# SunBangjie/FYP-BidirectionalPathTracer

Measured on AMD Instinct MI355X. Metric: Mrays/s + RMSE vs the scalar oracle, BDPT pass, Sponza-class scene 1920x1080 depth 8, higher is better.
Workload: dtype f32

## Files before the change

### fyp-bidirectionalpathtracer_amd/csrc/device_scene.hpp

```cpp
#pragma once
#include "device_math.hpp"
#include "kernels.h"

namespace bdpt {
#define BD __device__ __forceinline__

struct f4 {
  float x, y, z, w;
};
BD f4 lerp4(f4 a, f4 b, float s) {
  return f4{a.x + (b.x - a.x) * s, a.y + (b.y - a.y) * s, a.z + (b.z - a.z) * s, a.w + (b.w - a.w) * s};
}
typedef __attribute__((address_space(1))) const uint32_t gU32;
typedef __attribute__((address_space(1), aligned(4))) const unsigned long long gU64a4;
BD void texelRow(const uint8_t* px, uint32_t w, int iy, int ix0, int ix1, uint32_t& a, uint32_t& b) {
  gU32* row = (gU32*)px + (size_t)iy * w;
  const unsigned long long q = *(gU64a4*)(row + ix0);
  a = (uint32_t)q;
  b = (uint32_t)(q >> 32);
  if (ix1 != ix0 + 1) b = row[ix1];
}
BD f4 texel(const SceneDev& S, const TexDev& t, uint32_t p) {
  f4 r;
  if (t.srgb) {
    r.x = S.sc->srgbLut[p & 0xffu];
    r.y = S.sc->srgbLut[(p >> 8) & 0xffu];
    r.z = S.sc->srgbLut[(p >> 16) & 0xffu];
  } else {
    r.x = (float)(p & 0xffu) / 255.0f;
    r.y = (float)((p >> 8) & 0xffu) / 255.0f;
    r.z = (float)((p >> 16) & 0xffu) / 255.0f;
  }
  r.w = (float)(p >> 24) / 255.0f;
  return r;
}
BD f4 sampleBilinearT(const SceneDev& S, const TexDev& t, float u, float v) {
  float x = u * (float)t.w - 0.5f;
  float y = v * (float)t.h - 0.5f;
  float x0 = floorf(x), y0 = floorf(y);
  float fx = x - x0, fy = y - y0;
  int ix0 = wrapT((int)x0, (int)t.w, (t.pow2 & kTexPow2W) != 0u), iy0 = wrapT((int)y0, (int)t.h, (t.pow2 & kTexPow2H) != 0u);
  int ix1 = wrapNext(ix0, (int)t.w), iy1 = wrapNext(iy0, (int)t.h);
  uint32_t p00, p10, p01, p11;
  texelRow(t.px, t.w, iy0, ix0, ix1, p00, p10);
  texelRow(t.px, t.w, iy1, ix0, ix1, p01, p11);
  f4 t00 = texel(S, t, p00), t10 = texel(S, t, p10);
  f4 t01 = texel(S, t, p01), t11 = texel(S, t, p11);
  return lerp4(lerp4(t00, t10, fx), lerp4(t01, t11, fx), fy);
}
BD f4 sampleBilinear(const SceneDev& S, int texId, float u, float v) { return sampleBilinearT(S, S.textures[texId], u, v); }
BD f4 sampleTexture(const SceneDev& S, int texId, float u, float v, f4 factor, uint32_t mode) {
  if (mode == BDPT_CHANNEL_UNUSED) return f4{0, 0, 0, 0};
  if (mode == BDPT_CHANNEL_CONST || texId < 0) return factor;
  return sampleBilinear(S, texId, u, v);
}
BD f4 sampleTextureT(const SceneDev& S, const TexDev& t, int texId, float u, float v, f4 factor, uint32_t mode) {
  if (mode == BDPT_CHANNEL_UNUSED) return f4{0, 0, 0, 0};
  if (mode == BDPT_CHANNEL_CONST || texId < 0) return factor;
  return sampleBilinearT(S, t, u, v);
}

struct MatDev {
  f4 baseColor, specular;
  f3 emissive;
  float alphaThreshold, IoR;
  uint32_t flags;
  int texBase, texSpec, texEmis, texNorm;
};
BD MatDev loadMaterial(const SceneDev& S, uint32_t id) {
  const float4* m = reinterpret_cast<const float4*>(S.materials + id);
  float4 a = m[0], b = m[1], c = m[2], d = m[3];
  MatDev r;
  r.baseColor = f4{a.x, a.y, a.z, a.w};
  r.specular = f4{b.x, b.y, b.z, b.w};
  r.emissive = mk(c.x, c.y, c.z);
  r.alphaThreshold = c.w;
  r.IoR = d.x;
  r.flags = __float_as_uint(d.y);
  uint32_t t0 = __float_as_uint(d.z), t1 = __float_as_uint(d.w);
  r.texBase = (int)(int16_t)(t0 & 0xffffu);
  r.texSpec = (int)(int16_t)(t0 >> 16);
  r.texEmis = (int)(int16_t)(t1 & 0xffffu);
  r.texNorm = (int)(int16_t)(t1 >> 16);
  return r;
}

BD uint32_t alphaQuad(const float4& a2, const float4& a3, float u, float v, float& fx, float& fy) {
  const int tw = (int)__float_as_uint(a2.y), th = (int)__float_as_uint(a2.z);
  const uint32_t pow2 = __float_as_uint(a2.w);
  gU32* px = (gU32*)(((unsigned long long)__float_as_uint(a3.y) << 32) | (unsigned long long)__float_as_uint(a3.x));
  const float x = u * (float)tw - 0.5f, y = v * (float)th - 0.5f;
  const float x0 = floorf(x), y0 = floorf(y);
  fx = x - x0;
  fy = y - y0;
  const int ix0 = wrapT((int)x0, tw, (pow2 & kTexPow2W) != 0u), iy0 = wrapT((int)y0, th, (pow2 & kTexPow2H) != 0u);
  return px[(size_t)iy0 * tw + (size_t)ix0];
}
BD bool alphaTestFails(const SceneDev& S, uint32_t rec, float bu, float bv) {
  const float4* r = S.alphaRecs + (size_t)rec * 4;
  const float4 a0 = r[0], a1 = r[1], a2 = r[2], a3 = r[3];
  const uint32_t mode = __float_as_uint(a2.x);
  float alpha = 0.0f;
  if (mode == 1u) {
    alpha = a1.w;
  } else if (mode == 2u) {
    float u = 0, v = 0;
    const float b0 = 1.0f - bu - bv;
    u += a0.x * b0;
    v += a0.y * b0;
    u += a0.z * bu;
    v += a0.w * bu;
    u += a1.x * bv;
    v += a1.y * bv;
    float fx, fy;
    const uint32_t q = alphaQuad(a2, a3, u, v, fx, fy);
    const float t00 = (float)(q & 0xffu) / 255.0f, t10 = (float)((q >> 8) & 0xffu) / 255.0f;
    const float t01 = (float)((q >> 16) & 0xffu) / 255.0f, t11 = (float)(q >> 24) / 255.0f;
    const float top = t00 + (t10 - t00) * fx, bot = t01 + (t11 - t01) * fx;
    alpha = top + (bot - top) * fy;
  }
  return alpha < a1.z;
}

struct AlphaIn {
  float4 a0, a1, a2, a3;
};
BD void alphaTexels(const AlphaIn& r, float bu, float bv, bool run, float& fx, float& fy, float& t00, float& t10, float& t01, float& t11) {
  fx = fy = t00 = t10 = t01 = t11 = 0.0f;
  if (!run || __float_as_uint(r.a2.x) != 2u) return;
  float u = 0, v = 0;
  const float b0 = 1.0f - bu - bv;
  u += r.a0.x * b0;
  v += r.a0.y * b0;
  u += r.a0.z * bu;
  v += r.a0.w * bu;
  u += r.a1.x * bv;
  v += r.a1.y * bv;
  const uint32_t q = alphaQuad(r.a2, r.a3, u, v, fx, fy);
  t00 = (float)(q & 0xffu);
  t10 = (float)((q >> 8) & 0xffu);
  t01 = (float)((q >> 16) & 0xffu);
  t11 = (float)(q >> 24);
}
BD bool alphaVerdict(const AlphaIn& r, float fx, float fy, float t00, float t10, float t01, float t11) {
  const uint32_t mode = __float_as_uint(r.a2.x);
  float alpha = 0.0f;
  if (mode == 1u) {
    alpha = r.a1.w;
  } else if (mode == 2u) {
    const float w00 = t00 / 255.0f, w10 = t10 / 255.0f, w01 = t01 / 255.0f, w11 = t11 / 255.0f;
    const float top = w00 + (w10 - w00) * fx, bot = w01 + (w11 - w01) * fx;
    alpha = top + (bot - top) * fy;
  }
  return alpha < r.a1.z;
}
BD void alphaTestFails2(const SceneDev& S, bool need0, uint32_t rec0, float u0, float v0, bool need1, uint32_t rec1, float u1, float v1,
                        bool& fail0, bool& fail1) {
  AlphaIn r0, r1;
  r0.a0 = r0.a1 = r0.a2 = r0.a3 = r1.a0 = r1.a1 = r1.a2 = r1.a3 = make_float4(0.0f, 0.0f, 0.0f, 0.0f);
  if (need0) {
    const float4* p = S.alphaRecs + (size_t)rec0 * 4;
    r0.a0 = p[0];
    r0.a1 = p[1];
    r0.a2 = p[2];
    r0.a3 = p[3];
  }
  if (need1) {
    const float4* p = S.alphaRecs + (size_t)rec1 * 4;
    r1.a0 = p[0];
    r1.a1 = p[1];
    r1.a2 = p[2];
    r1.a3 = p[3];
  }
  float fx0, fy0, a00, a10, a01, a11, fx1, fy1, b00, b10, b01, b11;
  alphaTexels(r0, u0, v0, need0, fx0, fy0, a00, a10, a01, a11);
  alphaTexels(r1, u1, v1, need1, fx1, fy1, b00, b10, b01, b11);
  fail0 = need0 && alphaVerdict(r0, fx0, fy0, a00, a10, a01, a11);
  fail1 = need1 && alphaVerdict(r1, fx1, fy1, b00, b10, b01, b11);
}

struct Shading {
  f3 posW, V, N, diffuse, specular, emissive;
  float opacity, linearRoughness, roughness, IoR;
};
template <bool NMAP>
BD Shading shadeHit(const SceneDev& S, uint32_t prim, float bu, float bv, f3 camPosW) {
  const float4* r = S.shade + (size_t)prim * kShadeRecF4;
  const float4 r0 = r[0], r1 = r[1], r2 = r[2], r3 = r[3], r4 = r[4], r5 = r[5], r6 = r[6];
  const float b0 = 1.0f - bu - bv;
  float u = 0, v = 0;
  f3 normalW = mk(0), posW = mk(0);
  u += r1.z * b0;
  v += r1.w * b0;
  normalW = normalW + mk(r0.w, r1.x, r1.y) * b0;
  posW = posW + mk(r0.x, r0.y, r0.z) * b0;
  u += r3.z * bu;
  v += r3.w * bu;
  normalW = normalW + mk(r2.w, r3.x, r3.y) * bu;
  posW = posW + mk(r2.x, r2.y, r2.z) * bu;
  u += r5.z * bv;
  v += r5.w * bv;
  normalW = normalW + mk(r4.w, r5.x, r5.y) * bv;
  posW = posW + mk(r4.x, r4.y, r4.z) * bv;
  normalW = normalize(normalW);

  const uint32_t matId = __float_as_uint(r6.x);
  const MatDev m = loadMaterial(S, matId);
  const TexDev tBase = S.matTex[(size_t)matId * 4], tSpec = S.matTex[(size_t)matId * 4 + 1], tEmis = S.matTex[(size_t)matId * 4 + 2];
  Shading sd;
  f4 base = sampleTextureT(S, tBase, m.texBase, u, v, m.baseColor, BDPT_FLAG_DIFFUSE_TYPE(m.flags));
  sd.opacity = m.baseColor.w;
  sd.posW = posW;
  sd.V = normalize(camPosW - posW);
  sd.N = normalize(normalW);
  f4 spec = sampleTextureT(S, tSpec, m.texSpec, u, v, m.specular, BDPT_FLAG_SPECULAR_TYPE(m.flags));
  f3 baseRgb = mk(base.x, base.y, base.z);
  if (BDPT_FLAG_SHADING_MODEL(m.flags) == BDPT_SHADING_MODEL_METAL_ROUGH) {
    sd.diffuse = lerp3(baseRgb, mk(0), spec.z);
    sd.specular = lerp3(mk(0.04f), baseRgb, spec.z);
    sd.linearRoughness = spec.y;
  } else {
    sd.diffuse = baseRgb;
    sd.specular = mk(spec.x, spec.y, spec.z);
    sd.linearRoughness = 1.0f - spec.w;
  }
  sd.linearRoughness = maxf(0.08f, sd.linearRoughness);
  sd.roughness = sd.linearRoughness * sd.linearRoughness;
  f4 em = sampleTextureT(S, tEmis, m.texEmis, u, v, f4{m.emissive.x, m.emissive.y, m.emissive.z, 1.0f}, BDPT_FLAG_EMISSIVE_TYPE(m.flags));
  sd.emissive = mk(em.x, em.y, em.z);
  sd.IoR = m.IoR;
  const bool doubleSided = BDPT_FLAG_DOUBLE_SIDED(m.flags) != 0;
  if (NMAP) {
    const uint32_t mapType = BDPT_FLAG_NORMAL_MAP_TYPE(m.flags);
    if (mapType != BDPT_NORMAL_MAP_UNUSED && m.texNorm >= 0 && S.hasBitangents) {
      f3 bitW = mk(0);
      const float bw[3] = {b0, bu, bv};
#pragma unroll
      for (int i = 0; i < 3; i++) {
        uint32_t vi = S.indices[(size_t)prim * 3 + i];
        bitW = bitW + ld3(S.bitangents + (size_t)vi * 3) * bw[i];
      }
      bitW = normalize(bitW);
      f3 B = normalize(bitW - sd.N * dot(bitW, sd.N));
      f3 T = normalize(cross(B, sd.N));
      f4 mp = sampleBilinear(S, m.texNorm, u, v);
      f3 mapN;
      if (mapType == BDPT_NORMAL_MAP_RGB) {
        mapN = normalize(mk(mp.x, mp.y, mp.z) * 2.0f - mk(1.0f));
      } else {
        float nx = mp.x * 2.0f - 1.0f, ny = mp.y * 2.0f - 1.0f;
        float nz = saturate(mp.x * mp.x + mp.y * mp.y);
        nz = sqrtf(1.0f - nz);
        mapN = normalize(mk(nx, ny, nz));
      }
      sd.N = T * mapN.x + B * mapN.y + sd.N * mapN.z;
    }
  }
  float NdotV = dot(sd.N, sd.V);
  if (NdotV <= 0.0f && doubleSided) sd.N = -sd.N;
  return sd;
}

BD void primaryRay(const bdpt_camera& cam, const bdpt_gbuffer_params& gp, uint32_t x, uint32_t y, uint32_t W, uint32_t H, f3& o, f3& d) {
  const f3 U = ld3(cam.cameraU), V = ld3(cam.cameraV), Wv = ld3(cam.cameraW), camPos = ld3(cam.posW);
  float pcx = ((float)x + gp.pixelJitter[0]) / (float)W;
  float pcy = ((float)y + gp.pixelJitter[1]) / (float)H;
  float ndx = 2.0f * pcx + -1.0f;
  float ndy = -2.0f * pcy + 1.0f;
  f3 rayDir = U * ndx + V * ndy + Wv;
  rayDir = rayDir / length(Wv);
  f3 focalPoint = camPos + rayDir * gp.focalLen;
  uint32_t randSeed = initRand(x + y * W, gp.frameCount);
  float r0 = nextRand(randSeed);
  float r1 = nextRand(randSeed);
  float sn, cs;
  det_sincos2pi(r0, sn, cs);
  float lr = gp.lensRadius * r1;
  float lu = cs * lr, lv = sn * lr;
  f3 randomOrig = camPos + normalize(U) * lu + normalize(V) * lv;
  o = gp.useThinLens ? randomOrig : camPos;
  d = normalize(gp.useThinLens ? (focalPoint - randomOrig) : rayDir);
}

#undef BD
}
```

### fyp-bidirectionalpathtracer_amd/csrc/device_trace.hpp

```cpp
#pragma once
#include "bvh.h"
#include "device_scene.hpp"

namespace bdpt {
#define BD __device__ __forceinline__
#define BDPT_ONE_WAVE_PER_GROUP()               \
  do {                                          \
    if (blockDim.x != (unsigned)kWave) return;  \
  } while (0)

struct Hit {
  int prim;
  float t, u, v;
  uint32_t rec;
};

constexpr int kDone = (int)0x80000000;

struct TravState {
  f3 o, d, idir;
  uint32_t neg;
  float tmin, tmax;
  int cur, sp;
  Hit best;
// ... 266 lines not shown
}

template <int MODE, bool COUNT>
BD Hit traverse(const SceneDev& S, f3 o, f3 d, float tmin, float tmax, int* stk, uint32_t& nNodes, uint32_t& nTris) {
  uint32_t nAlpha = 0;
  TravState T;
  travInit(T, o, d, tmin, tmax);
  while (T.cur != kDone) {
    while (T.cur >= 0) {
      if (COUNT) nNodes++;
      nodeStep<(MODE != 2) ? 1 : 0>(S, T, stk);
    }
    if (T.cur == kDone) break;
    if (leafStep<MODE, COUNT>(S, T, nTris, nAlpha)) break;
    T.cur = travPop<kStackEntries>(S, T, stk);
  }
  return T.best;
}

constexpr uint32_t kNoHint = 0xFFFFFFFFu;
BD bool recOccludes(const SceneDev& S, uint32_t rec, f3 o, f3 d, float tmin, float tmax) {
  if (rec >= S.numRecs) return false;
  TravState T;
  travInit(T, o, d, tmin, tmax);
  if (T.cur == kDone) return false;
  const float4* tp = reinterpret_cast<const float4*>(S.recs) + (size_t)rec * kRecF4;
  const TriCand k = triGeom<2>(T, tp[0], tp[1], tp[2]);
  if (!k.ok) return false;
  if ((k.flags & 1u) && alphaTestFails(S, k.aux, k.u, k.v)) return false;
  return true;
}
BD uint32_t cubeTexel(f3 v, uint32_t res) {
  const float ax = fabsf(v.x), ay = fabsf(v.y), az = fabsf(v.z);
  uint32_t face;
  float ma, uc, vc;
  if (ax >= ay && ax >= az) {
    face = v.x < 0.0f ? 1u : 0u;
    ma = ax;
    uc = v.y;
    vc = v.z;
  } else if (ay >= az) {
    face = v.y < 0.0f ? 3u : 2u;
    ma = ay;
    uc = v.x;
    vc = v.z;
  } else {
    face = v.z < 0.0f ? 5u : 4u;
    ma = az;
    uc = v.x;
    vc = v.y;
  }
  if (!(ma > 0.0f)) return kNoHint;
  const float fr = (float)res;
  const float fu = (uc / ma * 0.5f + 0.5f) * fr, fv = (vc / ma * 0.5f + 0.5f) * fr;
  const uint32_t iu = fu >= fr ? res - 1u : (uint32_t)(fu < 0.0f ? 0.0f : fu), iv = fv >= fr ? res - 1u : (uint32_t)(fv < 0.0f ? 0.0f : fv);
  return (face * res + iv) * res + iu;
}
BD uint32_t lightHint(const SceneDev& S, int light, f3 lightPos, f3 pos) {
  if (!S.lightMap) return kNoHint;
  const uint32_t t = cubeTexel(pos - lightPos, S.lightMapRes);
  if (t == kNoHint) return kNoHint;
  return S.lightMap[(size_t)light * 6u * S.lightMapRes * S.lightMapRes + t];
}

BD void addCount(DevCounters* c, int idx, uint32_t n) {
  if (n) atomicAdd(&c->v[blockIdx.x % kCounterShards][idx], (unsigned long long)n);
}
BD void waveAddCount(DevCounters* c, int idx, uint32_t n) {
  uint32_t v = n;
#pragma unroll
  for (int off = 32; off > 0; off >>= 1) v += (uint32_t)__shfl_xor((int)v, off);
  if ((threadIdx.x & 63u) == 0u && v) atomicAdd(&c->v[blockIdx.x % kCounterShards][idx], (unsigned long long)v);
}

#ifndef BDPT_LEAF_WAIT
#define BDPT_LEAF_WAIT 1
#endif
#ifndef BDPT_LEAF_WAIT_FRAC8
#define BDPT_LEAF_WAIT_FRAC8 4
#endif
#ifndef BDPT_NODE_BURST
#define BDPT_NODE_BURST 3
#endif
#ifndef BDPT_REFILL_IDLE
#define BDPT_REFILL_IDLE 16
#endif
constexpr int kRefillIdle = BDPT_REFILL_IDLE;

struct RayQueue {
  const float* rays;
  uint32_t cap;
  uint32_t subCap;
  uint32_t numSub;
  const uint32_t* count;
  uint32_t* head;
};

template <bool COUNT>
__global__ __launch_bounds__(kWave) void trace_shadow_kernel(SceneDev S, RayQueue Q, uint8_t* __restrict__ vis, DevCounters* counters,
                                                             float shadowTmin) {
  BDPT_ONE_WAVE_PER_GROUP();
  __shared__ int s_stack[kStackLds * kWave];
  int* stk = s_stack + threadIdx.x;
  const int lane = (int)(threadIdx.x & 63u);
  bool has = false, exhausted = false;
  uint32_t rid = 0;
  TravState T;
  T.cur = kDone;
  uint32_t nNodes = 0, nTris = 0, nAlpha = 0;
  int maxSp = 0;
  uint32_t q = blockIdx.x % Q.numSub, tried = 0, chunkPos = 0, chunkEnd = 0, chunk = kFetchChunk;
  const uint32_t wavesPerList = (gridDim.x + Q.numSub - 1) / Q.numSub;
  for (;;) {
    const unsigned long long idleMask = __ballot(!has);
    const int idle = __popcll(idleMask);
    if (!exhausted && idle >= kRefillIdle) {
      while (chunkPos >= chunkEnd && !exhausted) {
        const uint32_t nq = Q.count[q * kCursorStride];
        uint32_t base = nq;
        if (__hip_atomic_load(&Q.head[q * kCursorStride], __ATOMIC_RELAXED, __HIP_MEMORY_SCOPE_AGENT) < nq) {
          uint32_t share = (nq / wavesPerList + kWave - 1) & ~(uint32_t)(kWave - 1);
          chunk = share < (uint32_t)kWave ? (uint32_t)kWave : (share > kFetchChunk ? kFetchChunk : share);
          if (lane == 0) base = atomicAdd(&Q.head[q * kCursorStride], chunk);
          base = (uint32_t)__builtin_amdgcn_readfirstlane((int)base);
        }
        if (base < nq) {
          chunkPos = base;
          chunkEnd = (base + chunk < nq) ? base + chunk : nq;
          tried = 0;
        } else {
          q = (q + 1 == Q.numSub) ? 0u : q + 1;
          if (++tried >= Q.numSub) exhausted = true;
        }
      }
      if (!exhausted) {
        const uint32_t avail = chunkEnd - chunkPos;
        const uint32_t take = ((uint32_t)idle < avail) ? (uint32_t)idle : avail;
        const uint32_t rank = (uint32_t)__popcll(idleMask & ((1ull << lane) - 1ull));
        if (!has && rank < take) {
          const uint32_t idx = q * Q.subCap + chunkPos + rank;
          rid = idx;
          const float* r = Q.rays + idx;
          const size_t c = Q.cap;
          travInit(T, mk(r[0], r[c], r[2 * c]),
                   mk(r[3 * c], r[4 * c], r[5 * c]), shadowTmin, r[6 * c]);
          has = true;
        }
        chunkPos += take;
      }
    }
    if (__ballot(has) == 0ull) break;
#if BDPT_LEAF_WAIT > 0
    if (has) {
#pragma unroll 1
      for (int k = 0; k < BDPT_NODE_BURST && T.cur >= 0; k++) {
        if (COUNT) nNodes++;
        nodeStep<0, kStackLds>(S, T, stk);
        if (COUNT) maxSp = T.sp > maxSp ? T.sp : maxSp;
      }
    }
    const unsigned long long waitMask = __ballot(has && T.cur < 0), nodeMask = __ballot(has && T.cur >= 0);
    const int waitNeed = (__popcll(waitMask | nodeMask) * BDPT_LEAF_WAIT_FRAC8 + 7) >> 3;
    if ((int)__popcll(waitMask) >= waitNeed || nodeMask == 0ull) {
      if (has && T.cur < 0) {
        bool finished = (T.cur == kDone);
        if (!finished) {
          finished = leafStep<2, COUNT>(S, T, nTris, nAlpha);
          if (!finished) {
            T.cur = travPop<kStackLds>(S, T, stk);
            finished = (T.cur == kDone);
          }
        }
        if (finished) {
          vis[rid] = (T.best.prim < 0) ? (uint8_t)1 : (uint8_t)0;
          has = false;
          T.cur = kDone;
        }
      }
    }
  }
#else
    if (has) {
      while (T.cur >= 0) {
        if (COUNT) nNodes++;
        nodeStep<0, kStackLds>(S, T, stk);
      }
      bool finished = (T.cur == kDone);
      if (!finished) {
        finished = leafStep<2, COUNT>(S, T, nTris, nAlpha);
        if (!finished) {
          T.cur = travPop<kStackLds>(S, T, stk);
          finished = (T.cur == kDone);
        }
      }
      if (finished) {
        vis[rid] = (T.best.prim < 0) ? (uint8_t)1 : (uint8_t)0;
        has = false;
        T.cur = kDone;
      }
    }
  }
#endif
  if (COUNT) {
    waveAddCount(counters, C_NODE_SHADOW, nNodes);
    waveAddCount(counters, C_TRI_SHADOW, nTris);
    waveAddCount(counters, C_ALPHA_SHADOW, nAlpha);
    if (maxSp > 0) atomicMax(&counters->v[blockIdx.x % kCounterShards][C_STACK_MAX], (unsigned long long)maxSp);
  }
}


#undef BD
}
```

### fyp-bidirectionalpathtracer_amd/csrc/kernels.h

```cpp
#pragma once
#include <hip/hip_runtime.h>
#include <stdint.h>

#include "../../include/bdpt.h"
#include "texture_planes.h"

namespace bdpt {

constexpr int kWave = 64;
#ifndef KSTACK
#define KSTACK 32
#endif
constexpr int kStackEntries = KSTACK;
#ifndef BDPT_STACK_LDS
#define BDPT_STACK_LDS 24
#endif
constexpr int kStackLds = BDPT_STACK_LDS < KSTACK ? BDPT_STACK_LDS : KSTACK;
constexpr int kMaxPersistentPerCU = 32;
constexpr int kStackOvfRows = KSTACK - kStackLds;
constexpr int kShadeRecF4 = 7;
constexpr uint32_t kNoRay = 0xFFFFFFFFu;
constexpr uint32_t kNumSubQueues = 32;
#ifndef BDPT_FETCH_CHUNK
#define BDPT_FETCH_CHUNK 256
#endif
constexpr uint32_t kFetchChunk = BDPT_FETCH_CHUNK;
constexpr uint32_t kCursorStride = 32;
constexpr uint32_t kCursorBlock = kNumSubQueues * kCursorStride;
#ifndef BDPT_RAY_SUBQUEUES
#define BDPT_RAY_SUBQUEUES 32
#endif
constexpr uint32_t kNumRaySubQueues = BDPT_RAY_SUBQUEUES;
constexpr uint32_t kRayCursorBlock = kNumRaySubQueues * kCursorStride;
constexpr uint32_t kCounterShards = 64;

enum : int { F_COL = 0, F_POS = 3, F_N = 6, F_V = 9, F_DIF = 12, F_SPEC = 15, F_ROUGH = 18, F_ISSPEC = 19, F_PDF = 20, NF = 21 };
constexpr int NF4 = 6;
enum : int { PATH_EYE = 0, PATH_LIGHT = 1 };
enum : int { RAY_TERMS = 0, RAY_PAIRS = 1 };

struct TexDev {
  const uint8_t* px;
  uint32_t w, h, srgb, pow2;
};

struct SceneConst {
  bdpt_light lights[BDPT_MAX_LIGHTS];
  float srgbLut[256];
};

struct SceneDev {
  const uint4* recs;
  const float4* shade;
  const float* bitangents;
  const uint32_t* indices;
  const bdpt_material* materials;
  const TexDev* textures;
  const TexDev* matTex;
  const SceneConst* sc;
  uint32_t numLights;
  uint32_t hasBitangents;
  uint32_t numRecs;
  const float4* alphaRecs;
  int* stackOvf;
  uint32_t stackOvfStride;
  const uint32_t* lightMap;
  uint32_t lightMapRes;
};

struct DevCounters {
  unsigned long long v[kCounterShards][32];
};
enum : int {
  C_RAYS_PRIMARY = 0, C_RAYS_EYE, C_RAYS_LIGHT, C_RAYS_NEE, C_RAYS_SPLAT, C_RAYS_CONNECT,
  C_NODE_CLOSEST, C_TRI_CLOSEST, C_NODE_SHADOW, C_TRI_SHADOW, C_PIX_VALID, C_SPLATS, C_RAYS_LAZY,
  C_STACK_MAX,
  C_ALPHA_CLOSEST, C_ALPHA_SHADOW,
  C_HINT_NEE, C_HINT_SPLAT
};

inline __host__ __device__ uint32_t numConnectPairs(uint32_t D) {
  uint32_t n = 0;
  for (uint32_t t = 2; t <= D; t++) n += (t < D - 1) ? t : (D - 1);
  return n;
}

struct PathBuf {
  float* v;
  float* rayDir;
  const uint32_t* pix;
  uint32_t* seedE;
  uint32_t* seedL;
  uint8_t* eyeLast;
  uint8_t* lightLast;
  uint8_t* lightReal;
  uint32_t* queue[3];
  uint32_t pathSubCap;
  uint32_t* qcount;
  uint32_t* qhead;
  float* rayQ;
  float* rayContrib;
  uint8_t* rayVis;
// ... 226 lines not shown
```

### fyp-bidirectionalpathtracer_amd/csrc/kernels.hip

```cpp
#include "kernels.h"

#include <algorithm>
#include <type_traits>

#include "device_area.hpp"
#include "device_connect.hpp"
#include "device_math.hpp"
#include "device_motion.hpp"
#include "device_scene.hpp"
#include "device_trace.hpp"
#include "launch.hpp"

namespace bdpt {

#define BD __device__ __forceinline__

BD void wavePush(bool active, uint32_t value, uint32_t* items, uint32_t* count, uint32_t subCap, uint32_t q = 0xffffffffu) {
  unsigned long long mask = __ballot(active);
  if (mask == 0ull) return;
  const int lane = (int)(threadIdx.x & 63u);
  const int leader = __ffsll((long long)mask) - 1;
  if (q == 0xffffffffu) q = blockIdx.x % kNumSubQueues;
  uint32_t base = 0;
  if (lane == leader) base = atomicAdd(&count[q * kCursorStride], (uint32_t)__popcll(mask));
// ... 235 lines not shown
      v.rough = roughness;
      v.isSpec = isSpec;
      v.pdf = pdf;
      storeVtx(P, PATH_EYE, 1, p, v);
      float* rd = P.rayDir + (size_t)(PATH_EYE * 3) * P.Np + p;
      rd[0] = outDir.x;
      rd[P.Np] = outDir.y;
      rd[2 * (size_t)P.Np] = outDir.z;

      const float areaW = AREA ? areaTotal(A) : 0.0f;
      const int lightsCount = (int)S.numLights + ((AREA && areaW > 0.0f) ? 1 : 0);
      int index = (int)(nextRand(seed) * (float)lightsCount);
      if (index > lightsCount - 1) index = lightsCount - 1;
      if (GROUPS) Gr.lightIdx[p] = (uint8_t)index;
      f3 lightDir;
      Vtx lv = zeroVtx();
      if (AREA && index == (int)S.numLights) {
        f3 n;
        lv.pos = areaLightStart(S, A, areaW, seed, n, lightDir, lv.color).pos;
      } else {
        const bdpt_light& l = S.sc->lights[index];
        if (l.type == BDPT_LIGHT_DIRECTIONAL)
          lightDir = ld3(l.dirW);
        else
          lightDir = sampleUnitSphere(seed);
        lightDir = getCosHemisphereSample(seed, lightDir);
        lv.pos = ld3(l.posW);
        lv.color = ld3(l.intensity);
      }
      lv.pdf = 1.0f / (float)lightsCount;
      storeVtx(P, PATH_LIGHT, 0, p, lv);
      float* rl = P.rayDir + (size_t)(PATH_LIGHT * 3) * P.Np + p;
      rl[0] = lightDir.x;
      rl[P.Np] = lightDir.y;
      rl[2 * (size_t)P.Np] = lightDir.z;
      P.seedL[p] = seed;

      const uint8_t D = (uint8_t)F.p.maxDepth;
      P.eyeLast[p] = D < 1 ? 1 : D;
      P.lightLast[p] = D;
      P.lightReal[p] = D;
      const bool em = (er > 0.0f) || (eg > 0.0f) || (eb > 0.0f);
      if (active) out4[pix] = em ? make_float4(0.0f + er, 0.0f + eg, 0.0f + eb, 0.0f + ea) : make_float4(0, 0, 0, 0);
    }
  }
  wavePush(geom, p, P.queue[0], P.qcount, P.pathSubCap);
  if (MASKED) wavePush(geom && active, p, M.eye, M.eyeCount, P.pathSubCap);
}
template <bool GGX, FrameKind V>
__global__ __launch_bounds__(kWave) void init_paths_kernel(SceneDev S, FrameDev F, PathBuf P, FrameArg<V> A) {
  BDPT_ONE_WAVE_PER_GROUP();
  initPathsLane<GGX, V == FrameKind::Groups, V == FrameKind::Masked>(S, F, P, groupOf(A), maskOf(A));
}
template <bool GGX, FrameKind V>
__global__ __launch_bounds__(kWave) void init_paths_area_kernel(SceneDev S, FrameDev F, PathBuf P, FrameArg<V> A, AreaDev E) {
  BDPT_ONE_WAVE_PER_GROUP();
  initPathsLane<GGX, V == FrameKind::Groups, V == FrameKind::Masked, true>(S, F, P, groupOf(A), maskOf(A), E);
}

constexpr uint32_t kPoolEntries = 128;
#ifndef BDPT_WALK_ORDER
#define BDPT_WALK_ORDER 1
#endif
#ifndef BDPT_WALK_SHADE_MIN
#define BDPT_WALK_SHADE_MIN 64
#endif
#ifndef BDPT_WALK_LEAF_WAIT
#define BDPT_WALK_LEAF_WAIT 1
#endif
#ifndef BDPT_WALK_NODE_BURST
#define BDPT_WALK_NODE_BURST 3
#endif
#ifndef BDPT_WALK_CHUNK
#define BDPT_WALK_CHUNK 64
#endif
#ifndef BDPT_WALK_REFILL
#define BDPT_WALK_REFILL BDPT_REFILL_IDLE
#endif
BD uint32_t packPath(uint32_t p, int path, int k) { return p | ((uint32_t)path << 24) | ((uint32_t)k << 25); }

#ifndef BDPT_WALK_WAVES_PER_EU
#define BDPT_WALK_WAVES_PER_EU 4
#endif
#ifndef BDPT_WALK_STACK_LDS
#define BDPT_WALK_STACK_LDS kStackEntries
#endif
constexpr int kWalkStackLds = BDPT_WALK_STACK_LDS;
constexpr uint32_t kParkedMiss = 1u << 30;
template <bool GGX, bool COUNT, bool EXT, bool MASKED>
__global__ __launch_bounds__(kWave) __attribute__((amdgpu_waves_per_eu(BDPT_WALK_WAVES_PER_EU, 8))) void walk_kernel(
    SceneDev S, FrameDev F, PathBuf P, uint32_t* __restrict__ head, FrameArg<MASKED ? FrameKind::Masked : FrameKind::Plain> mask) {
  BDPT_ONE_WAVE_PER_GROUP();
  __shared__ int s_stack[kWalkStackLds * kWave];
  __shared__ uint4 s_pool[kPoolEntries];
  const MaskDev& M = maskOf(mask);
  int* stk = s_stack + threadIdx.x;
  const int lane = (int)(threadIdx.x & 63u);
  const unsigned long long laneBelow = (1ull << lane) - 1ull;
  const int D = (int)F.p.maxDepth;
  const bool fromLobe = (F.p.flags & BDPT_PARAM_SPECULAR_FROM_LOBE) != 0;
  const uint32_t firstV = (D >= 2) ? 0u : kNumSubQueues, numV = 2u * kNumSubQueues - firstV;
  bool trav = false;
  uint32_t id = 0;
  TravState T;
  travInit(T, mk(0), mk(0), F.p.minT, 1.0e38f);
  T.cur = kDone;
  uint32_t nNodes = 0, nTris = 0, nAlpha = 0;
  uint32_t nEye = 0, nLight = 0, nParked = 0, nReady = 0;
  uint32_t vq = firstV + blockIdx.x % numV, tried = 0, chunkPos = 0, chunkEnd = 0, chunk = BDPT_WALK_CHUNK;
  bool exhausted = false;
  const uint32_t wavesPerList = (gridDim.x + numV - 1) / numV;
  for (;;) {
    unsigned long long travMask = __ballot(trav);
    const bool flush = (travMask == 0ull) && nReady == 0 && exhausted && nParked > 0;
    if (nParked >= (uint32_t)BDPT_WALK_SHADE_MIN || flush) {
      const uint32_t n = nParked < (uint32_t)kWave ? nParked : (uint32_t)kWave;
      nParked -= n;
      const bool act = (uint32_t)lane < n;
      uint4 rec = make_uint4(0, 0, 0, 0);
      if (act) rec = s_pool[nParked + (uint32_t)lane];
      __syncthreads();
      const uint32_t p = rec.x & 0xffffffu;
      const int path = (int)((rec.x >> 24) & 1u), k = (int)((rec.x >> 25) & 31u);
      nEye += (uint32_t)__popcll(__ballot(act && path == PATH_EYE));
      nLight += (uint32_t)__popcll(__ballot(act && path == PATH_LIGHT));
      bool survive = false;
      f3 L = mk(0);
      if (act) {
        const bool miss = EXT ? (rec.x & kParkedMiss) != 0u : (int)rec.y < 0;
        const int prim = miss ? -1 : (int)rec.y;
        const f3 o = ldPlane3(P, path, k, F_POS, p);
        f3 found = mk(0);
        bool haveFound = false;
        if (prim >= 0) {
          const uint32_t seed = (path == PATH_EYE) ? P.seedE[p] : P.seedL[p];
          const f3 thr = ldPlane3(P, path, k, F_COL, p);
          Shading sd = shadeHit<false>(S, (uint32_t)prim, __uint_as_float(rec.z), __uint_as_float(rec.w), o);
          float pdf;
          bool isSpec;
          f3 w = sampleBRDF<GGX>(seed, sd.N, sd.N, sd.V, sd.diffuse, sd.specular, sd.roughness, fromLobe, L, pdf, isSpec);
          Vtx v;
          v.color = thr * w;
          v.pos = sd.posW;
          v.N = sd.N;
          v.V = sd.V;
          v.dif = sd.diffuse;
          v.spec = sd.specular;
          v.rough = sd.roughness;
          v.isSpec = isSpec;
          v.pdf = pdf;
          storeVtx(P, path, k + 1, p, v);
          survive = (k + 2 <= D);
          if (EXT && path == PATH_EYE && (F.p.flags & BDPT_PARAM_EMISSIVE_HITS) &&
              (sd.emissive.x > 0.0f || sd.emissive.y > 0.0f || sd.emissive.z > 0.0f)) {
            found = thr * sd.emissive;
            haveFound = true;
          }
        } else {
          if (EXT && path == PATH_EYE && (F.p.flags & BDPT_PARAM_ENV_ON_MISS)) {
            const f3 dir = mk(__uint_as_float(rec.y), __uint_as_float(rec.z), __uint_as_float(rec.w));
            const f3 env = F.envMap ? envLookup(F.envMap, F.envW, F.envH, dir) : ld3(F.envColor);
            found = ldPlane3(P, path, k, F_COL, p) * env;
            haveFound = true;
          }
          Vtx g = zeroVtx();
          if (path == PATH_EYE && k == 1) {
            g.pos = o;
          } else {
            loadSurf(P, path, k, p, g);
            g.V = ldPlane3(P, path, k, F_V, p);
            if (path == PATH_LIGHT && k == 0) g.pdf = 0.0f;
          }
          g.color = mk(0);
          storeVtx(P, path, k + 1, p, g);
          if (path == PATH_EYE) {
            P.eyeLast[p] = (uint8_t)(k + 1);
          } else {
            P.lightLast[p] = (uint8_t)(k + 1);
            P.lightReal[p] = (uint8_t)k;
          }
        }
        if (MASKED && haveFound && M.mask[P.pix[p]] == 0) haveFound = false;
        if (EXT && haveFound) {
          f3 term = clampVec(found / (float)(k + 1), F.p.clampUpper);
          if (isnan3(term)) term = mk(0);
          float4* out4 = reinterpret_cast<float4*>(F.out);
          const size_t pix = P.pix[p];
          float4 acc = out4[pix];
          acc.x = acc.x + term.x;
          acc.y = acc.y + term.y;
          acc.z = acc.z + term.z;
          acc.w = acc.w + 1.0f;
          out4[pix] = acc;
        }
      }
      const unsigned long long sm = __ballot(survive);
      if (survive) {
        const uint32_t slot = kPoolEntries - 1u - nReady - (uint32_t)__popcll(sm & laneBelow);
        s_pool[slot] = make_uint4(packPath(p, path, k + 1), __float_as_uint(L.x), __float_as_uint(L.y), __float_as_uint(L.z));
      }
      nReady += (uint32_t)__popcll(sm);
      __builtin_amdgcn_fence(__ATOMIC_RELEASE, "workgroup");
      __syncthreads();
    }
    const int empty = 64 - __popcll(travMask);
    if ((empty >= BDPT_WALK_REFILL || travMask == 0ull) && (nReady > 0 || !exhausted)) {
      const unsigned long long emptyMask = ~travMask;
      const uint32_t rank = (uint32_t)__popcll(emptyMask & laneBelow);
      const uint32_t fromReady = ((uint32_t)empty < nReady) ? (uint32_t)empty : nReady;
      bool got = false;
      uint32_t nid = 0;
      f3 dir = mk(0);
      if (!trav && rank < fromReady) {
        const uint4 r = s_pool[kPoolEntries - nReady + rank];
        nid = r.x;
        dir = mk(__uint_as_float(r.y), __uint_as_float(r.z), __uint_as_float(r.w));
        got = true;
      }
      __syncthreads();
      nReady -= fromReady;
      uint32_t want = (uint32_t)empty - fromReady;
      uint32_t taken = fromReady;
      while (want > 0 && !exhausted) {
        while (chunkPos >= chunkEnd && !exhausted) {
          const uint32_t* counts = (MASKED && vq < kNumSubQueues) ? M.walkEyeCount : P.qcount;
          const uint32_t nq = counts[(vq % kNumSubQueues) * kCursorStride];
          uint32_t base = nq;
          if (__hip_atomic_load(&head[vq * kCursorStride], __ATOMIC_RELAXED, __HIP_MEMORY_SCOPE_AGENT) < nq) {
            uint32_t share = (nq / wavesPerList + 15u) & ~15u;
            chunk = share < 16u ? 16u : (share > (uint32_t)BDPT_WALK_CHUNK ? (uint32_t)BDPT_WALK_CHUNK : share);
            if (lane == 0) base = atomicAdd(&head[vq * kCursorStride], chunk);
            base = (uint32_t)__builtin_amdgcn_readfirstlane((int)base);
          }
          if (base < nq) {
            chunkPos = base;
            chunkEnd = (base + chunk < nq) ? base + chunk : nq;
            tried = 0;
          } else {
            vq = (vq + 1 == 2u * kNumSubQueues) ? firstV : vq + 1;
            if (++tried >= numV) exhausted = true;
          }
        }
        if (exhausted) break;
        const uint32_t avail = chunkEnd - chunkPos;
        const uint32_t take = (want < avail) ? want : avail;
        if (!trav && !got && rank >= taken && rank < taken + take) {
          const uint32_t* items = (MASKED && vq < kNumSubQueues) ? M.walkEye : P.queue[0];
          const uint32_t p = items[(vq % kNumSubQueues) * P.pathSubCap + chunkPos + (rank - taken)];
          const int path = (int)(vq / kNumSubQueues);
          const float* rd = P.rayDir + (size_t)(path * 3) * P.Np + p;
          nid = packPath(p, path, (path == PATH_EYE) ? 1 : 0);
          dir = mk(rd[0], rd[P.Np], rd[2 * (size_t)P.Np]);
          got = true;
        }
        chunkPos += take;
        taken += take;
        want -= take;
      }
      if (got) {
        id = nid;
        travInit(T, ldPlane3(P, (int)((nid >> 24) & 1u), (int)(nid >> 25), F_POS, nid & 0xffffffu), dir, F.p.minT, 1.0e38f);
        trav = true;
      }
      travMask = __ballot(trav);
    }
    if (travMask == 0ull) {
      if (nParked == 0 && nReady == 0 && exhausted) break;
      continue;
    }
    bool finished = false;
#if BDPT_WALK_LEAF_WAIT > 0
    if (trav) {
#pragma unroll 1
      for (int kk = 0; kk < BDPT_WALK_NODE_BURST && T.cur >= 0; kk++) {
        if (COUNT) nNodes++;
        nodeStep<BDPT_WALK_ORDER, kWalkStackLds>(S, T, stk);
      }
    }
    {
      const unsigned long long waitMask = __ballot(trav && T.cur < 0), nodeMask = __ballot(trav && T.cur >= 0);
      const int waitNeed = (__popcll(waitMask | nodeMask) * BDPT_LEAF_WAIT_FRAC8 + 7) >> 3;
      if ((int)__popcll(waitMask) >= waitNeed || nodeMask == 0ull) {
        if (trav && T.cur < 0) {
          finished = (T.cur == kDone);
          if (!finished) {
            finished = leafStep<0, COUNT>(S, T, nTris, nAlpha);
            if (!finished) {
              T.cur = travPop<kWalkStackLds>(S, T, stk);
              finished = (T.cur == kDone);
            }
          }
        }
      }
    }
#else
    if (trav) {
      while (T.cur >= 0) {
        if (COUNT) nNodes++;
        nodeStep<BDPT_WALK_ORDER, kWalkStackLds>(S, T, stk);
      }
      finished = (T.cur == kDone);
      if (!finished) {
        finished = leafStep<0, COUNT>(S, T, nTris, nAlpha);
        if (!finished) {
          T.cur = travPop<kWalkStackLds>(S, T, stk);
          finished = (T.cur == kDone);
        }
      }
    }
#endif
    const unsigned long long finMask = __ballot(finished);
    if (finMask) {
      if (finished) {
        const bool miss = T.best.prim < 0;
        s_pool[nParked + (uint32_t)__popcll(finMask & laneBelow)] =
            (EXT && miss) ? make_uint4(id | kParkedMiss, __float_as_uint(T.d.x), __float_as_uint(T.d.y), __float_as_uint(T.d.z))
                          : make_uint4(id, (uint32_t)T.best.prim, __float_as_uint(T.best.u), __float_as_uint(T.best.v));
        trav = false;
      }
      nParked += (uint32_t)__popcll(finMask);
      __syncthreads();
    }
  }
  if (lane == 0) {
    if (nEye) atomicAdd(&F.counters->v[blockIdx.x % kCounterShards][C_RAYS_EYE], (unsigned long long)nEye);
    if (nLight) atomicAdd(&F.counters->v[blockIdx.x % kCounterShards][C_RAYS_LIGHT], (unsigned long long)nLight);
  }
  if (COUNT) {
    waveAddCount(F.counters, C_NODE_CLOSEST, nNodes);
    waveAddCount(F.counters, C_TRI_CLOSEST, nTris);
    waveAddCount(F.counters, C_ALPHA_CLOSEST, nAlpha);
  }
}

BD float evalGWithoutVPos(f3 posA, f3 nA, f3 posB, f3 nB) {
  const f3 vecAB = posB - posA;
  const float invLengthAB = 1.0f / length(vecAB);
  const f3 dirAB = vecAB * invLengthAB;
  const float cosA = fabsf(dot(nA, dirAB));
  const float cosB = fabsf(dot(nB, dirAB));
  return cosA * cosB * invLengthAB * invLengthAB;
}

__global__ __launch_bounds__(kWave) void mis_prefix_kernel(FrameDev F, PathBuf P) {
  BDPT_ONE_WAVE_PER_GROUP();
  bool act = false;
  uint32_t i = 0;
  if (!queueChunk(P.qcount, P.pathSubCap, act, i)) return;
  if (!act) return;
  const uint32_t p = P.queue[0][i];
  const int D = (int)F.p.maxDepth;
  const int eyeLast = P.eyeLast[p], lightLast = P.lightLast[p];
  f3 prevPos = ld3(F.cam.posW), prevN = normalize(ld3(F.cam.cameraW));
  float pE = 1.0f;
  P.misE[p] = pE;
  for (int x = 1; x <= D; x++) {
    f3 pos = mk(0), N = mk(0);
    float pdf = 0.0f;
    if (x <= eyeLast) {
      pos = ldPlane3(P, PATH_EYE, x, F_POS, p);
// ... 1071 lines not shown
```

### fyp-bidirectionalpathtracer_amd/csrc/trace_rays.hip

```cpp
#include "kernels.h"

#include "device_math.hpp"
#include "device_query.hpp"
#include "device_scene.hpp"
#include "device_trace.hpp"
#include "launch.hpp"

namespace bdpt {

template <int MODE>
__global__ __launch_bounds__(kWave) void trace_rays_kernel(SceneDev S, const float4* __restrict__ rays, uint32_t cap,
                                                           const uint32_t* count, unsigned long long* cursor,
                                                           float4* __restrict__ hits, uint8_t* __restrict__ vis) {
  BDPT_ONE_WAVE_PER_GROUP();
  __shared__ int s_stack[kStackLds * kWave];
  int* stk = s_stack + threadIdx.x;
  const int lane = (int)(threadIdx.x & 63u);
  const uint32_t n = itemCount(cap, count);
  const uint32_t share = (n / gridDim.x + kWave - 1) & ~(uint32_t)(kWave - 1);
  const uint32_t chunk = share < (uint32_t)kWave ? (uint32_t)kWave : (share > kFetchChunk ? kFetchChunk : share);
  bool has = false, exhausted = false;
  uint32_t rid = 0, chunkPos = 0, chunkEnd = 0;
  uint32_t nTris = 0, nAlpha = 0;
  TravState T;
  T.cur = kDone;
  for (;;) {
    const unsigned long long idleMask = __ballot(!has);
    const int idle = __popcll(idleMask);
    if (!exhausted && idle >= kRefillIdle) {
      if (chunkPos >= chunkEnd) {
        unsigned long long base = 0;
        if (lane == 0) base = atomicAdd(cursor, (unsigned long long)chunk);
        base = ((unsigned long long)(uint32_t)__builtin_amdgcn_readfirstlane((int)(base >> 32)) << 32) |
               (uint32_t)__builtin_amdgcn_readfirstlane((int)(uint32_t)base);
        if (base < n) {
          chunkPos = (uint32_t)base;
          chunkEnd = (base + chunk < n) ? (uint32_t)(base + chunk) : n;
        } else {
          exhausted = true;
        }
      }
      if (!exhausted) {
        const uint32_t avail = chunkEnd - chunkPos;
        const uint32_t take = ((uint32_t)idle < avail) ? (uint32_t)idle : avail;
        const uint32_t rank = (uint32_t)__popcll(idleMask & ((1ull << lane) - 1ull));
        if (!has && rank < take) {
          rid = chunkPos + rank;
          const float4 a = rays[(size_t)rid * 2], b = rays[(size_t)rid * 2 + 1];
          travInit(T, mk(a.x, a.y, a.z), mk(b.x, b.y, b.z), a.w, b.w);
          has = true;
        }
        chunkPos += take;
      }
    }
    if (__ballot(has) == 0ull) break;
#if BDPT_LEAF_WAIT > 0
    if (has) {
#pragma unroll 1
      for (int k = 0; k < BDPT_NODE_BURST && T.cur >= 0; k++) nodeStep<(MODE != 2) ? 1 : 0, kStackLds>(S, T, stk);
    }
    const unsigned long long waitMask = __ballot(has && T.cur < 0), nodeMask = __ballot(has && T.cur >= 0);
    const int waitNeed = (__popcll(waitMask | nodeMask) * BDPT_LEAF_WAIT_FRAC8 + 7) >> 3;
    const bool leafPhase = (int)__popcll(waitMask) >= waitNeed || nodeMask == 0ull;
#else
    if (has)
      while (T.cur >= 0) nodeStep<(MODE != 2) ? 1 : 0, kStackLds>(S, T, stk);
    const bool leafPhase = true;
#endif
    if (leafPhase && has && T.cur < 0) {
      bool finished = (T.cur == kDone);
      if (!finished) {
        finished = leafStep<MODE, false>(S, T, nTris, nAlpha);
        if (!finished) {
          T.cur = travPop<kStackLds>(S, T, stk);
          finished = (T.cur == kDone);
        }
      }
      if (finished) {
        if (MODE == 2) {
          vis[rid] = (T.best.prim < 0) ? (uint8_t)1 : (uint8_t)0;
        } else {
          const bool hit = T.best.prim >= 0;
          hits[rid] = make_float4(hit ? T.best.t : 0.0f, hit ? T.best.u : 0.0f, hit ? T.best.v : 0.0f, __int_as_float(T.best.prim));
        }
        has = false;
        T.cur = kDone;
      }
    }
  }
  if (lane == 0) {
    __threadfence();
    if (atomicAdd(&cursor[1], 1ull) == (unsigned long long)gridDim.x - 1ull) {
      cursor[0] = 0ull;
      cursor[1] = 0ull;
    }
  }
}

void launchTraceRays(const SceneDev& S, const float4* rays, uint32_t cap, const uint32_t* count, unsigned long long* cursor, int mode,
                     float4* hits, uint8_t* vis, LaunchGrids& G, int numCUs, hipStream_t st) {
  if (!cap) return;
  static constexpr decltype(&trace_rays_kernel<0>) kByMode[3] = {trace_rays_kernel<0>, trace_rays_kernel<1>, trace_rays_kernel<2>};
  const auto kernel = kByMode[mode];
  uint32_t& g = G.rays[mode];
  if (!g) g = persistentGrid(kernel, numCUs);
  const uint32_t need = wavesFor(cap);
  launchWave(kernel, g < need ? g : need, st, S, rays, cap, count, cursor, hits, vis);
}

}
```

Before: 4851.

## Stage sRGB LUT in LDS and add a wave-uniform fast path for LDS-only traversal stack

The walk kernel now copies the 256-entry sRGB lookup table into shared memory at launch and passes it through templated texture sampling, so texture decodes read LDS instead of global memory. A new nodeBurst helper checks, via a wave ballot, whether any lane's stack pointer could pass the LDS portion within the burst. When none can, it runs nodeStep with the full stack bound, which is meant to skip per-push overflow checks. The walk kernel's LDS stack is also reduced from the full stack size to 28 entries, with overflow rows sized to match. The costs are an extra ballot per burst, more LDS per wave, and a global overflow path for deep stacks in the walk kernel, which may affect occupancy and spill traffic.

```diff
diff --git a/fyp-bidirectionalpathtracer_amd/csrc/device_scene.hpp b/fyp-bidirectionalpathtracer_amd/csrc/device_scene.hpp
--- a/fyp-bidirectionalpathtracer_amd/csrc/device_scene.hpp
+++ b/fyp-bidirectionalpathtracer_amd/csrc/device_scene.hpp
@@ -20,12 +20,15 @@
   b = (uint32_t)(q >> 32);
   if (ix1 != ix0 + 1) b = row[ix1];
 }
-BD f4 texel(const SceneDev& S, const TexDev& t, uint32_t p) {
+typedef __attribute__((address_space(3))) const float ldsF32;
+BD const float* globalSrgb(const SceneDev& S) { return S.sc->srgbLut; }
+template <class Lut>
+BD f4 texel(Lut srgb, const TexDev& t, uint32_t p) {
   f4 r;
   if (t.srgb) {
-    r.x = S.sc->srgbLut[p & 0xffu];
-    r.y = S.sc->srgbLut[(p >> 8) & 0xffu];
-    r.z = S.sc->srgbLut[(p >> 16) & 0xffu];
+    r.x = srgb[p & 0xffu];
+    r.y = srgb[(p >> 8) & 0xffu];
+    r.z = srgb[(p >> 16) & 0xffu];
   } else {
     r.x = (float)(p & 0xffu) / 255.0f;
     r.y = (float)((p >> 8) & 0xffu) / 255.0f;
@@ -34,7 +37,8 @@
   r.w = (float)(p >> 24) / 255.0f;
   return r;
 }
-BD f4 sampleBilinearT(const SceneDev& S, const TexDev& t, float u, float v) {
+template <class Lut>
+BD f4 sampleBilinearT(Lut srgb, const TexDev& t, float u, float v) {
   float x = u * (float)t.w - 0.5f;
   float y = v * (float)t.h - 0.5f;
   float x0 = floorf(x), y0 = floorf(y);
@@ -44,20 +48,15 @@
   uint32_t p00, p10, p01, p11;
   texelRow(t.px, t.w, iy0, ix0, ix1, p00, p10);
   texelRow(t.px, t.w, iy1, ix0, ix1, p01, p11);
-  f4 t00 = texel(S, t, p00), t10 = texel(S, t, p10);
-  f4 t01 = texel(S, t, p01), t11 = texel(S, t, p11);
+  f4 t00 = texel(srgb, t, p00), t10 = texel(srgb, t, p10);
+  f4 t01 = texel(srgb, t, p01), t11 = texel(srgb, t, p11);
   return lerp4(lerp4(t00, t10, fx), lerp4(t01, t11, fx), fy);
 }
-BD f4 sampleBilinear(const SceneDev& S, int texId, float u, float v) { return sampleBilinearT(S, S.textures[texId], u, v); }
-BD f4 sampleTexture(const SceneDev& S, int texId, float u, float v, f4 factor, uint32_t mode) {
+template <class Lut>
+BD f4 sampleTextureT(Lut srgb, const TexDev& t, int texId, float u, float v, f4 factor, uint32_t mode) {
   if (mode == BDPT_CHANNEL_UNUSED) return f4{0, 0, 0, 0};
   if (mode == BDPT_CHANNEL_CONST || texId < 0) return factor;
-  return sampleBilinear(S, texId, u, v);
-}
-BD f4 sampleTextureT(const SceneDev& S, const TexDev& t, int texId, float u, float v, f4 factor, uint32_t mode) {
-  if (mode == BDPT_CHANNEL_UNUSED) return f4{0, 0, 0, 0};
-  if (mode == BDPT_CHANNEL_CONST || texId < 0) return factor;
-  return sampleBilinearT(S, t, u, v);
+  return sampleBilinearT(srgb, t, u, v);
 }
 
 struct MatDev {
@@ -183,8 +182,8 @@
   f3 posW, V, N, diffuse, specular, emissive;
   float opacity, linearRoughness, roughness, IoR;
 };
-template <bool NMAP>
-BD Shading shadeHit(const SceneDev& S, uint32_t prim, float bu, float bv, f3 camPosW) {
+template <bool NMAP, class Lut>
+BD Shading shadeHitLut(const SceneDev& S, Lut srgb, uint32_t prim, float bu, float bv, f3 camPosW) {
   const float4* r = S.shade + (size_t)prim * kShadeRecF4;
   const float4 r0 = r[0], r1 = r[1], r2 = r[2], r3 = r[3], r4 = r[4], r5 = r[5], r6 = r[6];
   const float b0 = 1.0f - bu - bv;
@@ -208,12 +207,12 @@
   const MatDev m = loadMaterial(S, matId);
   const TexDev tBase = S.matTex[(size_t)matId * 4], tSpec = S.matTex[(size_t)matId * 4 + 1], tEmis = S.matTex[(size_t)matId * 4 + 2];
   Shading sd;
-  f4 base = sampleTextureT(S, tBase, m.texBase, u, v, m.baseColor, BDPT_FLAG_DIFFUSE_TYPE(m.flags));
+  f4 base = sampleTextureT(srgb, tBase, m.texBase, u, v, m.baseColor, BDPT_FLAG_DIFFUSE_TYPE(m.flags));
   sd.opacity = m.baseColor.w;
   sd.posW = posW;
   sd.V = normalize(camPosW - posW);
   sd.N = normalize(normalW);
-  f4 spec = sampleTextureT(S, tSpec, m.texSpec, u, v, m.specular, BDPT_FLAG_SPECULAR_TYPE(m.flags));
+  f4 spec = sampleTextureT(srgb, tSpec, m.texSpec, u, v, m.specular, BDPT_FLAG_SPECULAR_TYPE(m.flags));
   f3 baseRgb = mk(base.x, base.y, base.z);
   if (BDPT_FLAG_SHADING_MODEL(m.flags) == BDPT_SHADING_MODEL_METAL_ROUGH) {
     sd.diffuse = lerp3(baseRgb, mk(0), spec.z);
@@ -226,7 +225,7 @@
   }
   sd.linearRoughness = maxf(0.08f, sd.linearRoughness);
   sd.roughness = sd.linearRoughness * sd.linearRoughness;
-  f4 em = sampleTextureT(S, tEmis, m.texEmis, u, v, f4{m.emissive.x, m.emissive.y, m.emissive.z, 1.0f}, BDPT_FLAG_EMISSIVE_TYPE(m.flags));
+  f4 em = sampleTextureT(srgb, tEmis, m.texEmis, u, v, f4{m.emissive.x, m.emissive.y, m.emissive.z, 1.0f}, BDPT_FLAG_EMISSIVE_TYPE(m.flags));
   sd.emissive = mk(em.x, em.y, em.z);
   sd.IoR = m.IoR;
   const bool doubleSided = BDPT_FLAG_DOUBLE_SIDED(m.flags) != 0;
@@ -243,7 +242,7 @@
       bitW = normalize(bitW);
       f3 B = normalize(bitW - sd.N * dot(bitW, sd.N));
       f3 T = normalize(cross(B, sd.N));
-      f4 mp = sampleBilinear(S, m.texNorm, u, v);
+      f4 mp = sampleBilinearT(srgb, S.textures[m.texNorm], u, v);
       f3 mapN;
       if (mapType == BDPT_NORMAL_MAP_RGB) {
         mapN = normalize(mk(mp.x, mp.y, mp.z) * 2.0f - mk(1.0f));
@@ -259,6 +258,10 @@
   float NdotV = dot(sd.N, sd.V);
   if (NdotV <= 0.0f && doubleSided) sd.N = -sd.N;
   return sd;
+}
+template <bool NMAP>
+BD Shading shadeHit(const SceneDev& S, uint32_t prim, float bu, float bv, f3 camPosW) {
+  return shadeHitLut<NMAP>(S, globalSrgb(S), prim, bu, bv, camPosW);
 }
 
 BD void primaryRay(const bdpt_camera& cam, const bdpt_gbuffer_params& gp, uint32_t x, uint32_t y, uint32_t W, uint32_t H, f3& o, f3& d) {
diff --git a/fyp-bidirectionalpathtracer_amd/csrc/device_trace.hpp b/fyp-bidirectionalpathtracer_amd/csrc/device_trace.hpp
--- a/fyp-bidirectionalpathtracer_amd/csrc/device_trace.hpp
+++ b/fyp-bidirectionalpathtracer_amd/csrc/device_trace.hpp
@@ -372,6 +372,28 @@
 #ifndef BDPT_NODE_BURST
 #define BDPT_NODE_BURST 3
 #endif
+template <int ORDER, int KL, int BURST, bool COUNT>
+BD void nodeBurst(const SceneDev& S, TravState& T, int* stk, bool has, uint32_t& nNodes, int& maxSp) {
+  static_assert(ORDER >= 0 && ORDER <= 2, "the margin below is worked out for nodeStep's three child orders");
+  constexpr int kMargin = 3 * BURST + (ORDER == 2 ? 1 : 0);
+  if (KL < kStackEntries && __ballot(has && T.sp > KL - kMargin) != 0ull) {
+    if (has) {
+#pragma unroll 1
+      for (int k = 0; k < BURST && T.cur >= 0; k++) {
+        if (COUNT) nNodes++;
+        nodeStep<ORDER, KL>(S, T, stk);
+        if (COUNT) maxSp = T.sp > maxSp ? T.sp : maxSp;
+      }
+    }
+  } else if (has) {
+#pragma unroll 1
+    for (int k = 0; k < BURST && T.cur >= 0; k++) {
+      if (COUNT) nNodes++;
+      nodeStep<ORDER, kStackEntries>(S, T, stk);
+      if (COUNT) maxSp = T.sp > maxSp ? T.sp : maxSp;
+    }
+  }
+}
 #ifndef BDPT_REFILL_IDLE
 #define BDPT_REFILL_IDLE 16
 #endif
@@ -441,14 +463,7 @@
     }
     if (__ballot(has) == 0ull) break;
 #if BDPT_LEAF_WAIT > 0
-    if (has) {
-#pragma unroll 1
-      for (int k = 0; k < BDPT_NODE_BURST && T.cur >= 0; k++) {
-        if (COUNT) nNodes++;
-        nodeStep<0, kStackLds>(S, T, stk);
-        if (COUNT) maxSp = T.sp > maxSp ? T.sp : maxSp;
-      }
-    }
+    nodeBurst<0, kStackLds, BDPT_NODE_BURST, COUNT>(S, T, stk, has, nNodes, maxSp);
     const unsigned long long waitMask = __ballot(has && T.cur < 0), nodeMask = __ballot(has && T.cur >= 0);
     const int waitNeed = (__popcll(waitMask | nodeMask) * BDPT_LEAF_WAIT_FRAC8 + 7) >> 3;
     if ((int)__popcll(waitMask) >= waitNeed || nodeMask == 0ull) {
diff --git a/fyp-bidirectionalpathtracer_amd/csrc/kernels.h b/fyp-bidirectionalpathtracer_amd/csrc/kernels.h
--- a/fyp-bidirectionalpathtracer_amd/csrc/kernels.h
+++ b/fyp-bidirectionalpathtracer_amd/csrc/kernels.h
@@ -16,8 +16,12 @@
 #define BDPT_STACK_LDS 24
 #endif
 constexpr int kStackLds = BDPT_STACK_LDS < KSTACK ? BDPT_STACK_LDS : KSTACK;
+#ifndef BDPT_WALK_STACK_LDS
+#define BDPT_WALK_STACK_LDS 28
+#endif
+constexpr int kWalkStackLds = BDPT_WALK_STACK_LDS < KSTACK ? BDPT_WALK_STACK_LDS : KSTACK;
 constexpr int kMaxPersistentPerCU = 32;
-constexpr int kStackOvfRows = KSTACK - kStackLds;
+constexpr int kStackOvfRows = KSTACK - (kStackLds < kWalkStackLds ? kStackLds : kWalkStackLds);
 constexpr int kShadeRecF4 = 7;
 constexpr uint32_t kNoRay = 0xFFFFFFFFu;
 constexpr uint32_t kNumSubQueues = 32;
diff --git a/fyp-bidirectionalpathtracer_amd/csrc/kernels.hip b/fyp-bidirectionalpathtracer_amd/csrc/kernels.hip
--- a/fyp-bidirectionalpathtracer_amd/csrc/kernels.hip
+++ b/fyp-bidirectionalpathtracer_amd/csrc/kernels.hip
@@ -341,10 +341,6 @@
 #ifndef BDPT_WALK_WAVES_PER_EU
 #define BDPT_WALK_WAVES_PER_EU 4
 #endif
-#ifndef BDPT_WALK_STACK_LDS
-#define BDPT_WALK_STACK_LDS kStackEntries
-#endif
-constexpr int kWalkStackLds = BDPT_WALK_STACK_LDS;
 constexpr uint32_t kParkedMiss = 1u << 30;
 template <bool GGX, bool COUNT, bool EXT, bool MASKED>
 __global__ __launch_bounds__(kWave) __attribute__((amdgpu_waves_per_eu(BDPT_WALK_WAVES_PER_EU, 8))) void walk_kernel(
@@ -352,6 +348,11 @@
   BDPT_ONE_WAVE_PER_GROUP();
   __shared__ int s_stack[kWalkStackLds * kWave];
   __shared__ uint4 s_pool[kPoolEntries];
+  __shared__ float s_srgb[256];
+#pragma unroll
+  for (int i = 0; i < 256; i += kWave) s_srgb[i + (int)threadIdx.x] = S.sc->srgbLut[i + (int)threadIdx.x];
+  __syncthreads();
+  ldsF32* const srgb = (ldsF32*)s_srgb;
   const MaskDev& M = maskOf(mask);
   int* stk = s_stack + threadIdx.x;
   const int lane = (int)(threadIdx.x & 63u);
@@ -394,7 +395,7 @@
         if (prim >= 0) {
           const uint32_t seed = (path == PATH_EYE) ? P.seedE[p] : P.seedL[p];
           const f3 thr = ldPlane3(P, path, k, F_COL, p);
-          Shading sd = shadeHit<false>(S, (uint32_t)prim, __uint_as_float(rec.z), __uint_as_float(rec.w), o);
+          Shading sd = shadeHitLut<false>(S, srgb, (uint32_t)prim, __uint_as_float(rec.z), __uint_as_float(rec.w), o);
           float pdf;
           bool isSpec;
           f3 w = sampleBRDF<GGX>(seed, sd.N, sd.N, sd.V, sd.diffuse, sd.specular, sd.roughness, fromLobe, L, pdf, isSpec);
@@ -529,12 +530,9 @@
     }
     bool finished = false;
 #if BDPT_WALK_LEAF_WAIT > 0
-    if (trav) {
-#pragma unroll 1
-      for (int kk = 0; kk < BDPT_WALK_NODE_BURST && T.cur >= 0; kk++) {
-        if (COUNT) nNodes++;
-        nodeStep<BDPT_WALK_ORDER, kWalkStackLds>(S, T, stk);
-      }
+    {
+      int maxSp = 0;
+      nodeBurst<BDPT_WALK_ORDER, kWalkStackLds, BDPT_WALK_NODE_BURST, COUNT>(S, T, stk, trav, nNodes, maxSp);
     }
     {
       const unsigned long long waitMask = __ballot(trav && T.cur < 0), nodeMask = __ballot(trav && T.cur >= 0);
diff --git a/fyp-bidirectionalpathtracer_amd/csrc/trace_rays.hip b/fyp-bidirectionalpathtracer_amd/csrc/trace_rays.hip
--- a/fyp-bidirectionalpathtracer_amd/csrc/trace_rays.hip
+++ b/fyp-bidirectionalpathtracer_amd/csrc/trace_rays.hip
@@ -55,9 +55,10 @@
     }
     if (__ballot(has) == 0ull) break;
 #if BDPT_LEAF_WAIT > 0
-    if (has) {
-#pragma unroll 1
-      for (int k = 0; k < BDPT_NODE_BURST && T.cur >= 0; k++) nodeStep<(MODE != 2) ? 1 : 0, kStackLds>(S, T, stk);
+    {
+      uint32_t nNodes = 0;
+      int maxSp = 0;
+      nodeBurst<(MODE != 2) ? 1 : 0, kStackLds, BDPT_NODE_BURST, false>(S, T, stk, has, nNodes, maxSp);
     }
     const unsigned long long waitMask = __ballot(has && T.cur < 0), nodeMask = __ballot(has && T.cur >= 0);
     const int waitNeed = (__popcll(waitMask | nodeMask) * BDPT_LEAF_WAIT_FRAC8 + 7) >> 3;
```

Result: faster. 4916, median of 6 (+1.4%).
